# nihaomiao/CVPR23_LFDM

Measured on AMD Instinct MI355X. Metric: 40-frame 128x128 videos/sec (DDIM-100), higher is better.
Workload: dtype f32; 1 GPU; MUG 128x128, 40-frame DDIM-100 sample, batch=1 per GPU (BASELINE.json configs[1]); global_batch=1, frames=40, latent=32, image=128, sampler=DDIM-100 eta=1, cond_scale=1, parallelism=replicas x1 (videos sharded, no collective)

## Files before the change

cvpr23_lfdm_amd/_native.py:

```python
import ctypes as C
import os

_PKG_DIR = os.path.dirname(os.path.abspath(__file__))
HIP_LIB_PATH = os.environ.get("LFDM_HIP_LIB", os.path.join(_PKG_DIR, "liblfdm_hip.so"))

f32p = C.c_void_p
i32 = C.c_int
i64 = C.c_int64
f32 = C.c_float
sz = C.c_size_t
stream_t = C.c_void_p


class ConvParams(C.Structure):
    _fields_ = [
        ("src0", f32p), ("src1", f32p),
        ("c0", i32), ("c1", i32), ("ld0", i32), ("ld1", i32),
        ("n_img", i32), ("hi", i32), ("wi", i32),
        ("hq", i32), ("wq", i32),
        ("stride", i32), ("upsample", i32), ("pad_mode", i32),
        ("kh", i32), ("kw", i32), ("pad_y", i32), ("pad_x", i32),
        ("weight", f32p),
        ("cout", i32), ("coutp", i32),
        ("bias", f32p),
# ... 73 lines not shown
class WarpBwdParams(C.Structure):
    _fields_ = [
        ("src", f32p), ("dout", f32p), ("prev", f32p), ("dprev", f32p), ("dsrc_fix", C.c_void_p), ("amax_bits", C.c_void_p),
        ("dmaps", f32p), ("flow_x", f32p), ("flow_y", f32p), ("occ", f32p),
        ("n_img", i32), ("h", i32), ("w", i32), ("c", i32), ("fh", i32), ("fw", i32), ("n_div", i32), ("layout_cl", i32),
        ("fsn", i64),
        ("ld_src", i32), ("ld_dout", i32), ("ld_prev", i32), ("ld_dprev", i32),
        ("ss_n", i64), ("ss_c", i64), ("ss_h", i64), ("ss_w", i64), ("ds_n", i64), ("ds_c", i64), ("ds_h", i64), ("ds_w", i64),
        ("ps_n", i64), ("ps_c", i64), ("ps_h", i64), ("ps_w", i64), ("dps_n", i64), ("dps_c", i64), ("dps_h", i64), ("dps_w", i64),
    ]


class GridSampleParams(C.Structure):
    _fields_ = [
        ("x", f32p), ("grid", f32p), ("out", f32p), ("dout", f32p), ("dgrid", f32p),
        ("xs_n", i64), ("xs_c", i64), ("xs_h", i64), ("xs_w", i64), ("os_n", i64), ("os_c", i64), ("os_h", i64), ("os_w", i64),
        ("n_img", i32), ("channels", i32), ("h", i32), ("w", i32), ("ho", i32), ("wo", i32), ("n_div", i32), ("pad_mode", i32),
    ]


BN_TICKETS = 1024
OPTIM_PLAN_BYTES = 64

_SIGNATURES = {
    "lfdm_last_error": (C.c_char_p, []),
    "lfdm_abi_version": (i32, []),
    "lfdm_calib_mfma_f32": (i32, [f32p, i32, i32, stream_t]),
    "lfdm_conv2d_cl_f32": (i32, [C.POINTER(ConvParams), stream_t]),
    "lfdm_conv2d_cl_wino_bf16": (i32, [C.POINTER(ConvParams), C.c_void_p, stream_t]),
    "lfdm_conv2d_partial_bytes": (sz, [C.POINTER(ConvParams)]),
    "lfdm_conv2d_plan": (i32, [C.POINTER(ConvParams), C.POINTER(i32), C.POINTER(i32)]),
    "lfdm_conv2d_plan_slabs": (i32, [C.POINTER(ConvParams)]),
    "lfdm_conv2d_schedule": (i32, [C.POINTER(ConvParams)]),
    "lfdm_groupnorm_ws_bytes": (sz, [i32, i32, i32]),
    "lfdm_groupnorm_silu_cl_f32": (i32, [f32p, f32p, i32, i32, i32, i32, f32p, f32p, f32p, i32, f32p,
                                        f32, i32, C.c_void_p, sz, stream_t]),
    "lfdm_groupnorm_apply_cl_f32": (i32, [f32p, f32p, i32, i32, i32, i32, f32p, f32p, f32p, i32, f32p, f32, i32,
                                         f32p, i32, C.c_void_p, sz, stream_t]),
    "lfdm_layernorm_cl_f32": (i32, [f32p, f32p, i64, i32, f32p, f32, stream_t]),
    "lfdm_attention_cl_f32": (i32, [f32p, f32p, i32, i32, i32, i32, f32p, f32p, f32p, stream_t]),
    "lfdm_temporal_attention_fused_cl_f32": (i32, [f32p, i32, i32, f32p, f32p, i32, i32, i32, f32p, f32p, f32p, f32,
                                                  stream_t]),
    "lfdm_temporal_attention_fused_out_cl_f32": (i32, [f32p, i32, i32, f32p, f32p, f32p, i32, i32, i32, i32, f32p, f32p, f32p, f32,
                                                      stream_t]),
    "lfdm_linear_attention_lowres_cl_f32": (i32, [f32p, i32, i32, f32p, f32p, f32p, i32, i32, f32, stream_t]),
    "lfdm_attention_lowres_cl_f32": (i32, [f32p, i32, i32, f32p, f32p, f32p, i32, i32, i32, i32, f32p, f32p, f32p, f32, stream_t]),
    "lfdm_pack_wino_weight_f32": (i32, [f32p, i32, i32, i32, i32, i32, f32p, stream_t]),
    "lfdm_pack_wino4_weight_f32": (i32, [f32p, i32, i32, i32, i32, f32p, stream_t]),
    "lfdm_pack_wino_weight_bf16": (i32, [f32p, i32, i32, i32, i32, C.c_void_p, stream_t]),
    "lfdm_pack_conv_weight_f32": (i32, [f32p, i32, i32, i32, i64, i64, i32, f32p, stream_t]),
    "lfdm_lfae_motion_inputs_f32": (i32, [f32p, f32p, f32p, f32p, f32p, f32p, f32p, f32p, C.c_float, i32, i32, i32, i32, i32, i32,
                                          f32p, i32, f32p, stream_t]),
    "lfdm_lfae_region_stats_f32": (i32, [f32p, i32, i32, i32, i32, i32, C.c_float, f32p, f32p, f32p, f32p, f32p, f32p, stream_t]),
    "lfdm_svd2x2_sym_f32": (i32, [f32p, i64, f32p, f32p, stream_t]),
    "lfdm_lfae_motion_combine_f32": (i32, [f32p, i32, f32p, i32, i32, i32, f32p, f32p, stream_t]),
    "lfdm_conv2d_smalln_cl_f32": (i32, [f32p, i32, i32, i32, i32, i32, f32p, f32p, f32p, i32, i32, i32, i32, stream_t]),
    "lfdm_linear_attention_fused_ws_bytes": (sz, [i32, i32]),
    "lfdm_linear_attention_fused_cl_f32": (i32, [f32p, i32, i32, f32p, f32p, i32, i32, f32, C.c_void_p, sz, stream_t]),
    "lfdm_linear_attention_fused_out_cl_f32": (i32, [f32p, i32, i32, f32p, f32p, f32p, f32p, i32, i32, i32, f32, C.c_void_p, sz, stream_t]),
    "lfdm_linear_attention_ws_bytes": (sz, [i32]),
    "lfdm_linear_attention_cl_f32": (i32, [f32p, f32p, i32, i32, C.c_void_p, sz, stream_t]),
    "lfdm_linear_small_f32": (i32, [f32p, f32p, f32p, f32p, i32, i32, i32, i32, i32, i32, i32, i32, stream_t]),
    "lfdm_step_cond_f32": (i32, [f32p, f32p, C.c_void_p, f32p, i32, i32, stream_t]),
    "lfdm_sinusoidal_f32": (i32, [C.c_void_p, i32, f32p, f32p, i32, i32, i32, stream_t]),
    "lfdm_conv_planar_in_cl_f32": (i32, [f32p, i32, i32, i32, i32, i32, i32, f32p, i32, i32, i32,
                                        f32p, f32p, f32p, i32, i32, stream_t]),
# ... 121 lines not shown
```

cvpr23_lfdm_amd/csrc/conv_igemm.hip:

```cpp
#include <stdlib.h>

#include "lfdm_device.h"
#include "../../include/lfdm_hip.h"

namespace {

__device__ __forceinline__ bool src_pixel(const lfdm_conv_params& p, int img, int qy, int qx,
                                          int tap, int64_t& pix) {
  const int ky = tap / p.kw, kx = tap - ky * p.kw;
  int iy = qy * p.stride + ky - p.pad_y;
  int ix = qx * p.stride + kx - p.pad_x;
  const int H = p.upsample ? 2 * p.hi : p.hi;
  const int W = p.upsample ? 2 * p.wi : p.wi;
  if (p.pad_mode == 1) {
    if (iy < 0) iy = -iy;
    if (iy >= H) iy = 2 * (H - 1) - iy;
    if (ix < 0) ix = -ix;
    if (ix >= W) ix = 2 * (W - 1) - ix;
  } else if (iy < 0 || iy >= H || ix < 0 || ix >= W) {
    return false;
  }
  if (p.upsample) {
    iy >>= 1;
    ix >>= 1;
// ... 600 lines not shown
int splitk_col_chunks(const lfdm_conv_params& p, int64_t M) {
  const int c4n = p.coutp / 4;
  const int64_t rowblocks = (M + SPLITK_ROWS - 1) / SPLITK_ROWS;
  int gy = 1;
  while (rowblocks * gy < 256 && gy < 16) {
    const int cand = gy * 2;
    if (c4n % cand != 0) break;
    const int cw = c4n / cand;
    if (cw < 16) break;
    if (p.gn_partial) {
      const int cg4 = (p.cout / p.gn_groups) / 4;
      if (cw % cg4 != 0 || 256 % cw != 0) break;
    }
    gy = cand;
  }
  return gy;
}

template <int BM, int BN>
void launch_conv(const lfdm_conv_params& p, bool fast, bool simple, dim3 grid, hipStream_t stream) {
  dim3 block(256);
  if (fast && simple && p.ln_wsum) LFDM_LAUNCH((conv_igemm_kernel<BM, BN, true, true, true>), grid, block, 0, stream, p);
  else if (fast && simple) LFDM_LAUNCH((conv_igemm_kernel<BM, BN, true, true, false>), grid, block, 0, stream, p);
  else if (fast) LFDM_LAUNCH((conv_igemm_kernel<BM, BN, true, false, false>), grid, block, 0, stream, p);
  else LFDM_LAUNCH((conv_igemm_kernel<BM, BN, false, false, false>), grid, block, 0, stream, p);
}

}

int lfdm_conv_ksw_launch(const lfdm_conv_params& p, int bn, hipStream_t stream);
int lfdm_conv_wino_launch(const lfdm_conv_params& p, int bn, bool fuse_reduce, int bal_whole, hipStream_t stream);
int lfdm_conv_wino_bf16_launch(const lfdm_conv_params& p, const void* weight_bf16, int bn, bool fuse_reduce, int bal_whole, hipStream_t stream);
int lfdm_conv_pw_launch(const lfdm_conv_params& p, hipStream_t stream);
int lfdm_conv_wino4_launch(const lfdm_conv_params& p, hipStream_t stream);

namespace {

struct ConvPlan;
bool splitk_fused(const ConvPlan& pl, const lfdm_conv_params& p);
bool wino_fuse_geometry_ok(const lfdm_conv_params& p, int bn);
int wino_balance(const ConvPlan& pl, const lfdm_conv_params& p, int* extra_slabs);

struct ConvPlan {
  int kind;
  int bm, bn, ksplit;
  bool fast, simple;
};

int conv_force() {
  static int v = -2;
  if (v == -2) {
    const char* e = getenv("LFDM_CONV_FORCE");
    v = !e ? -1 : (e[0] == 'k' ? 1 : 0);
  }
  return v;
}

bool wino_enabled() {
  const char* e = getenv("LFDM_WINO");
  return !(e && e[0] == '0');
}

ConvPlan make_plan(const lfdm_conv_params& p) {
  ConvPlan pl;
  const int cin = p.c0 + p.c1;
  const int64_t M = (int64_t)p.n_img * p.hq * p.wq;
// ... 81 lines not shown
  if (ksw) {
    pl.kind = 1;
    pl.bm = 160;
    const int64_t mt = (M + 159) / 160 * (p.deconv4 ? 4 : 1);
    const int64_t t64 = mt * ((p.coutp + 63) / 64), t32 = mt * ((p.coutp + 31) / 32);
    pl.bn = (t64 >= 224 && p.coutp > 32) ? 64 : 32;
    int k = 1;
    if (t64 < 224 && t32 < 224) {
      k = (int)(256 / t32);
      if (k > nchunks / 4) k = nchunks / 4;
      if (k < 1) k = 1;
    }
    pl.ksplit = user_k >= 1 ? user_k : k;
  } else {
    pl.kind = 0;
    static const long wide_min = [] { const char* e = lfdm_knob("LFDM_IGEMM_WIDE_MIN"); return e ? atol(e) : 512l; }();
    const bool wide = p.coutp >= 128 && (M / 128) * (p.coutp / 128) >= wide_min;
    const bool small_m = M * (int64_t)((p.coutp + 63) / 64) < 128 * 512;
    pl.bm = wide ? 128 : (small_m ? 64 : 128);
    pl.bn = wide ? 128 : 64;
    int k = 1;
    const int64_t tiles = ((M + pl.bm - 1) / pl.bm) * ((p.coutp + pl.bn - 1) / pl.bn) * (p.deconv4 ? 4 : 1);
    if (tiles < 256 && nchunks >= 8) {
      k = (int)(512 / tiles);
      if (k > nchunks / 4) k = nchunks / 4;
      if (k > 16) k = 16;
      if (k < 1) k = 1;
    }
    pl.ksplit = user_k >= 1 ? user_k : k;
  }
  if (pl.ksplit > nchunks) pl.ksplit = nchunks;
  if (pl.ksplit < 1) pl.ksplit = 1;
  const int64_t pw_rows = (!p.ln_wsum && p.c0 + p.c1 <= 256 && p.coutp <= 128) ? 10240 : 1024;
  if (pwg_ok || (pw_ok && (pw_mode == 2 || M <= pw_rows || pl.ksplit > 1 || p.res_gn_partial))) {
    pl.kind = 3;
    pl.bm = 32;
    pl.bn = 32;
    pl.ksplit = 1;
  }
  return pl;
}

bool wino_fuse_geometry_ok(const lfdm_conv_params& p, int bn) {
  static const bool on = [] { const char* e = getenv("LFDM_WINO_FUSE_REDUCE"); return !(e && e[0] == '0'); }();
  if (!on || !p.tile_counters || p.deconv4 || bn != 32 || p.groups > 1 || p.pool2 || p.cout != p.coutp || p.ldo % 4 != 0 ||
      (((uintptr_t)p.out) & 15) != 0 ||
      (p.bias && (((uintptr_t)p.bias) & 15) != 0) ||
      (p.residual && (p.ldr % 4 != 0 || (((uintptr_t)p.residual) & 15) != 0)))
    return false;
  const int64_t ntiles = (int64_t)p.n_img * (p.hq / 2) * (p.wq / 2);
  return (int64_t)p.tile_counters_len >= ((ntiles + 31) / 32) * (p.coutp / 32);
}

bool splitk_fused(const ConvPlan& pl, const lfdm_conv_params& p) {
  if (pl.ksplit <= 1 || pl.kind != 2 || !wino_fuse_geometry_ok(p, pl.bn)) return false;
  const int64_t M = (int64_t)p.n_img * p.hq * p.wq;
  return (int64_t)pl.ksplit * M * p.coutp * 4 < (1ll << 32) - 64;
}

int wino_balance(const ConvPlan& pl, const lfdm_conv_params& p, int* extra_slabs) {
  if (extra_slabs) *extra_slabs = 0;
  static const bool on = [] { const char* e = getenv("LFDM_WINO_BALANCE"); return !(e && e[0] == '0'); }();
  static const bool fuse_on = [] { const char* e = getenv("LFDM_WINO_FUSE_REDUCE"); return !(e && e[0] == '0'); }();
  if (!on || !fuse_on || pl.kind != 2 || pl.bn != 32 || !p.tile_counters || p.deconv4 || p.groups > 1 || p.pool2 || p.cout != p.coutp || p.ldo % 4 != 0 ||
      (((uintptr_t)p.out) & 15) != 0 || (p.bias && (((uintptr_t)p.bias) & 15) != 0) ||
      (p.residual && (p.ldr % 4 != 0 || (((uintptr_t)p.residual) & 15) != 0)))
    return 0;
  if (pl.ksplit > 1 && !splitk_fused(pl, p)) return 0;
  const int64_t ntiles = (int64_t)p.n_img * (p.hq / 2) * (p.wq / 2);
  const int64_t T = ((ntiles + 31) / 32) * (p.coutp / 32);
  const int whole = 512, jobs = 640;
  if (T * pl.ksplit != jobs || (int64_t)p.tile_counters_len < T) return 0;
  const int nch = (p.c0 + p.c1) / 16;
  if (nch / pl.ksplit < 2) return 0;
  const int z_first = T - 1 >= whole ? 0 : (int)((whole - (T - 1) + T - 1) / T);
  const int extra = pl.ksplit - z_first;
  if (extra < 1) return 0;
  const int64_t M = (int64_t)p.n_img * p.hq * p.wq;
  if ((int64_t)(pl.ksplit + extra) * M * p.coutp * 4 >= (1ll << 32) - 64) return 0;
  if (extra_slabs) *extra_slabs = extra;
  return whole;
}

}

extern "C" int lfdm_conv2d_plan(const lfdm_conv_params* p, int* tile_rows, int* ksplit) {
  if (!p) return LFDM_EINVAL;
  const ConvPlan pl = make_plan(*p);
  if (tile_rows) *tile_rows = (pl.ksplit > 1 && !splitk_fused(pl, *p)) ? SPLITK_ROWS : pl.bm;
  if (ksplit) *ksplit = pl.ksplit;
  return LFDM_OK;
}

extern "C" int lfdm_conv2d_schedule(const lfdm_conv_params* p) {
  if (!p) return LFDM_EINVAL;
  return make_plan(*p).kind;
}

extern "C" size_t lfdm_conv2d_partial_bytes(const lfdm_conv_params* p) {
  if (!p) return 0;
  const ConvPlan pl = make_plan(*p);
  int extra = 0;
  wino_balance(pl, *p, &extra);
  if (pl.ksplit <= 1 && extra == 0) return 0;
  const size_t rows = (size_t)p->n_img * p->hq * p->wq;
  return ((size_t)(pl.ksplit + extra) * (p->deconv4 ? 4 : 1) * rows * p->coutp + (p->ln_wsum ? (size_t)pl.ksplit * rows * 2 : 0)) * sizeof(float) + 128;
}

extern "C" int lfdm_conv2d_plan_slabs(const lfdm_conv_params* p) {
  if (!p) return LFDM_EINVAL;
  const ConvPlan pl = make_plan(*p);
  int extra = 0;
  wino_balance(pl, *p, &extra);
  return pl.ksplit + extra;
}

namespace {

int conv2d_run(const lfdm_conv_params* pp, const void* wino_bf16, hipStream_t stream) {
  if (!pp) { lfdm_set_error("conv2d: null params"); return LFDM_EINVAL; }
  lfdm_conv_params p = *pp;
  if (!p.src0 || !p.weight || !p.out || p.c0 <= 0 || p.c1 < 0 || (p.c1 > 0 && !p.src1) ||
      p.n_img <= 0 || p.hq <= 0 || p.wq <= 0 || p.kh <= 0 || p.kw <= 0 || p.cout <= 0 ||
      (int64_t)p.n_img * p.hq * p.wq >= (1ll << 31) || p.coutp < p.cout || (p.coutp % 32) != 0 || p.stride <= 0 || p.out_scale <= 0 || p.ksplit < 0 ||
      p.ld0 < p.c0 || (p.c1 > 0 && p.ld1 < p.c1) || p.ldo < p.cout) {
    lfdm_set_error("conv2d: invalid geometry");
    return LFDM_EINVAL;
  }
  if (p.pad_mode == 1) {
    const int H = p.upsample ? 2 * p.hi : p.hi, W = p.upsample ? 2 * p.wi : p.wi;
    if (p.pad_y >= H || p.pad_x >= W || p.kh - 1 - p.pad_y >= H || p.kw - 1 - p.pad_x >= W) {
// ... 117 lines not shown
```

cvpr23_lfdm_amd/csrc/conv_pw.hip:

```cpp
#include <stdlib.h>

#include "lfdm_device.h"
#include "../../include/lfdm_hip.h"

namespace {

template <int TN, int KW, bool LN, bool GATHER = false>
__global__ __launch_bounds__(256) void conv_pw_kernel(lfdm_conv_params p, int gx, int ny) {
  constexpr int NW = 4 / KW;
  constexpr int LD = 36;
  __shared__ __attribute__((aligned(16))) float scratch[4 * 32 * LD];
  __shared__ float s_ln[2][4][32];
  constexpr int BN = (4 / KW) * TN * 32;
  __shared__ __attribute__((aligned(16))) float s_ga[BN], s_gb[BN];
  __shared__ float s_gstat[2][64];

  const int tid = threadIdx.x, lane = tid & 63;
  const int wave = lfdm_uniform(tid >> 6);
  const int wk = wave % KW, wn = wave / KW;
  const int id = blockIdx.x, slot = id >> 3;
  const int bx = (id & 7) + 8 * (slot / ny), by = slot % ny;
  if (bx >= gx) return;
  const int M = p.n_img * p.hq * p.wq;
  const int m0 = bx * 32;
// ... 199 lines not shown
    for (int g = 0; g < NW; ++g) {
      float4 v = *reinterpret_cast<const float4*>(scratch + (g * KW) * (32 * LD) + trow * LD + 4 * c4);
#pragma unroll
      for (int k = 1; k < KW; ++k) {
        const float4 u = *reinterpret_cast<const float4*>(scratch + (g * KW + k) * (32 * LD) + trow * LD + 4 * c4);
        v.x += u.x; v.y += u.y; v.z += u.z; v.w += u.w;
      }
      const int col = n0 + (g * TN + j) * 32 + 4 * c4;
      if (!vec_row || col >= p.cout) continue;
      if (LN) {
        const float4 ws = pre_w[g * TN + j];
        v.x = rstd * (v.x - mean * ws.x); v.y = rstd * (v.y - mean * ws.y);
        v.z = rstd * (v.z - mean * ws.z); v.w = rstd * (v.w - mean * ws.w);
      }
      {
        const float4 bb = pre_b[g * TN + j];
        float4 rr = pre_r[g * TN + j];
        if (p.res_gn_partial) {
          const float4 ga = *reinterpret_cast<const float4*>(s_ga + col - n0), gb = *reinterpret_cast<const float4*>(s_gb + col - n0);
          rr.x = silu_fast_(fmaf(rr.x, ga.x, gb.x)); rr.y = silu_fast_(fmaf(rr.y, ga.y, gb.y));
          rr.z = silu_fast_(fmaf(rr.z, ga.z, gb.z)); rr.w = silu_fast_(fmaf(rr.w, ga.w, gb.w));
        }
        v.x += bb.x + rr.x; v.y += bb.y + rr.y; v.z += bb.z + rr.z; v.w += bb.w + rr.w;
      }
      if (p.act) {
        v.x = apply_act(v.x, p.act); v.y = apply_act(v.y, p.act);
        v.z = apply_act(v.z, p.act); v.w = apply_act(v.w, p.act);
      }
      *reinterpret_cast<float4*>(p.out + (int64_t)orow * p.ldo + col) = v;
    }
  }
}

template <int TN, int KW>
void launch_pw(const lfdm_conv_params& p, int gx, int ny, hipStream_t stream) {
  const dim3 grid((unsigned)(((gx + 7) / 8) * 8 * ny)), block(256);
  if (p.kh * p.kw > 1) {
    if constexpr (TN <= 2 && KW == 4) LFDM_LAUNCH((conv_pw_kernel<TN, 4, false, true>), grid, block, 0, stream, p, gx, ny);
    return;
  }
  if (p.ln_wsum) LFDM_LAUNCH((conv_pw_kernel<TN, KW, true>), grid, block, 0, stream, p, gx, ny);
  else LFDM_LAUNCH((conv_pw_kernel<TN, KW, false>), grid, block, 0, stream, p, gx, ny);
}

int env_int(const char* name, int dflt) {
  const char* e = lfdm_knob(name);
  return e ? atoi(e) : dflt;
}

}

void lfdm_conv_pw_shape(const lfdm_conv_params& p, int* tn, int* kw) {
  const int K = p.kh * p.kw > 1 ? p.kh * p.kw * p.c0 : p.c0 + p.c1;
  const int64_t M = (int64_t)p.n_img * p.hq * p.wq;
  if (p.kh * p.kw > 1) {
    *tn = (p.coutp % 64 == 0 && ((M + 31) / 32) * (p.coutp / 64) >= 256) ? 2 : 1;
    *kw = 4;
    return;
  }
  int k = K % 128 == 0 ? 4 : K % 64 == 0 ? 2 : 1;
  const int fk = env_int("LFDM_PW_KW", 0);
  if ((fk == 1 || fk == 2 || fk == 4) && K % (32 * fk) == 0) k = fk;
  int t = (M <= 1024 && p.coutp >= 768 && p.coutp % ((4 / k) * 96) == 0) ? 3 : 1;
  const int ft = env_int("LFDM_PW_TN", 0);
  if (ft >= 1 && ft <= 3) t = ft;
  *tn = t;
  *kw = k;
}

int lfdm_conv_pw_launch(const lfdm_conv_params& p, hipStream_t stream) {
  int tn, kw;
  lfdm_conv_pw_shape(p, &tn, &kw);
  const int64_t M = (int64_t)p.n_img * p.hq * p.wq;
  const int gx = (int)((M + 31) / 32);
  const int bn = (4 / kw) * tn * 32;
  const int ny = (p.coutp + bn - 1) / bn;
#define LFDM_PW_CASE(T, W) if (tn == T && kw == W) launch_pw<T, W>(p, gx, ny, stream)
  LFDM_PW_CASE(1, 4); else LFDM_PW_CASE(2, 4); else LFDM_PW_CASE(3, 4);
  else LFDM_PW_CASE(1, 2); else LFDM_PW_CASE(2, 2); else LFDM_PW_CASE(3, 2);
  else LFDM_PW_CASE(1, 1); else LFDM_PW_CASE(2, 1); else LFDM_PW_CASE(3, 1);
#undef LFDM_PW_CASE
  return lfdm_check_launch("conv_pw");
}
```

cvpr23_lfdm_amd/csrc/lfdm_device.h:

```cpp
#pragma once
#include <stddef.h>
#include <stdint.h>
#include <type_traits>

#if defined(LFDM_EMU_BUILD)
#include "hip_emu.h"
typedef emu_f32x16 f32x16;
typedef emu_f32x4 f32x4;
#define LFDM_LAUNCH(kern, grid, block, smem, stream, ...) \
  emu::launch(grid, block, smem, [=]() { kern(__VA_ARGS__); })
static inline f32x16 mfma_32x32x2(float a, float b, f32x16 c) { return emu_mfma_32x32x2(a, b, c); }
static inline f32x4 mfma_16x16x4(float a, float b, f32x4 c) { return emu_mfma_16x16x4(a, b, c); }
static inline f32x4 mfma_4x4x1(float a, float b, f32x4 c) { return emu_mfma_4x4x1(a, b, c); }
struct lfdm_bf16x8 { uint16_t h[8]; };
static inline uint16_t lfdm_f32_to_bf16(float f) {
  uint32_t u;
  memcpy(&u, &f, 4);
  if ((u & 0x7fffffffu) > 0x7f800000u) return (uint16_t)((u >> 16) | 0x40u);
  u += 0x7fffu + ((u >> 16) & 1u);
  return (uint16_t)(u >> 16);
}
static inline float lfdm_bf16_to_f32(uint16_t h) {
  const uint32_t u = (uint32_t)h << 16;
  float f;
// ... 85 lines not shown
  float4 v = make_float4(0.f, 0.f, 0.f, 0.f);
  if ((uint64_t)off + 16u <= (uint64_t)b.bytes) memcpy(&v, b.base + off, 16);
  return v;
}
static inline float2 lfdm_buf_load_f2(lfdm_buf b, uint32_t off) {
  float2 v = make_float2(0.f, 0.f);
  if ((uint64_t)off + 8u <= (uint64_t)b.bytes) memcpy(&v, b.base + off, 8);
  return v;
}
#else
typedef __amdgpu_buffer_rsrc_t lfdm_buf;
typedef int lfdm_i32x4 __attribute__((ext_vector_type(4)));
__device__ __forceinline__ lfdm_buf lfdm_make_buf(const void* p, uint32_t bytes) {
  return __builtin_amdgcn_make_buffer_rsrc(const_cast<void*>(p), 0, (int)bytes, 0x00020000);
}
__device__ __forceinline__ float4 lfdm_buf_load_f4(lfdm_buf b, uint32_t off) {
  const lfdm_i32x4 v = __builtin_amdgcn_raw_buffer_load_b128(b, (int)off, 0, 0);
  float4 f;
  f.x = __int_as_float(v.x);
  f.y = __int_as_float(v.y);
  f.z = __int_as_float(v.z);
  f.w = __int_as_float(v.w);
  return f;
}
typedef int lfdm_i32x2 __attribute__((ext_vector_type(2)));
__device__ __forceinline__ float2 lfdm_buf_load_f2(lfdm_buf b, uint32_t off) {
  const lfdm_i32x2 v = __builtin_amdgcn_raw_buffer_load_b64(b, (int)off, 0, 0);
  return make_float2(__int_as_float(v.x), __int_as_float(v.y));
}
#endif
#define LFDM_BUF_OOB 0xFFFFFFF0u

#if defined(LFDM_EMU_BUILD)
static inline void lfdm_buf_store_f4_sc1(lfdm_buf b, uint32_t off, float4 v) {
  if ((uint64_t)off + 16u <= (uint64_t)b.bytes) memcpy(const_cast<char*>(b.base) + off, &v, 16);
}
static inline float4 lfdm_buf_load_f4_sc1(lfdm_buf b, uint32_t off) { return lfdm_buf_load_f4(b, off); }
#else
__device__ __forceinline__ void lfdm_buf_store_f4_sc1(lfdm_buf b, uint32_t off, float4 v) {
  lfdm_i32x4 d;
  d.x = __float_as_int(v.x); d.y = __float_as_int(v.y); d.z = __float_as_int(v.z); d.w = __float_as_int(v.w);
  __builtin_amdgcn_raw_buffer_store_b128(d, b, (int)off, 0, 16);
}
__device__ __forceinline__ float4 lfdm_buf_load_f4_sc1(lfdm_buf b, uint32_t off) {
  const lfdm_i32x4 v = __builtin_amdgcn_raw_buffer_load_b128(b, (int)off, 0, 16);
  float4 f;
  f.x = __int_as_float(v.x); f.y = __int_as_float(v.y); f.z = __int_as_float(v.z); f.w = __int_as_float(v.w);
  return f;
}
#endif

#if defined(LFDM_EMU_BUILD)
template <int OFF = 0> static inline void lfdm_gload_f4(f32x4& dst, const float* p) { memcpy(&dst, (const char*)p + OFF, 16); }
template <int N> static inline void lfdm_vmwait() {}
template <int N> static inline void lfdm_vmwait(f32x4&) {}
template <int N> static inline void lfdm_vmwait(f32x4&, f32x4&) {}
template <int N> static inline void lfdm_vmwait(f32x4&, f32x4&, f32x4&, f32x4&) {}
static inline void lfdm_tie(f32x4&) {}
static inline int lfdm_uniform(int v) { return v; }
#else
template <int OFF = 0>
__device__ __forceinline__ void lfdm_gload_f4(f32x4& dst, const float* p) {
  asm volatile("global_load_dwordx4 %0, %1, off offset:%2" : "=v"(dst) : "v"(p), "n"(OFF) : "memory");
}
template <int N> __device__ __forceinline__ void lfdm_vmwait() { asm volatile("s_waitcnt vmcnt(%0)" ::"n"(N) : "memory"); }
template <int N> __device__ __forceinline__ void lfdm_vmwait(f32x4& a) { asm volatile("s_waitcnt vmcnt(%1)" : "+v"(a) : "n"(N) : "memory"); }
// ... 99 lines not shown
```

cvpr23_lfdm_amd/ops.py:

```python
import ctypes as C

import torch

from . import _native
from ._native import ConvParams, WarpParams

ACT_NONE, ACT_RELU, ACT_SIGMOID, ACT_SILU, ACT_GELU = 0, 1, 2, 3, 4


def _lib():
    return _native.library()


def _stream(lib):
    if lib.kind == "hip":
        return C.c_void_p(torch.cuda.current_stream().cuda_stream)
    return None


def _p(t):
    return None if t is None else C.c_void_p(t.data_ptr())


def _chk(lib, *tensors):
# ... 306 lines not shown
        _chk(lib, gp, gg, gb)
        assert residual is not None and gg.numel() == cout == gb.numel() and gp.is_contiguous()
        p.res_gn_partial, p.res_gn_nchunk, p.res_gn_groups, p.res_gn_pixels = _p(gp), int(res_gn["nchunk"]), int(res_gn.get("groups", 8)), int(res_gn["pixels"])
        p.res_gn_gamma, p.res_gn_beta, p.res_gn_eps = _p(gg), _p(gb), float(res_gn.get("eps", 1e-5))
        keep_gn = keep_gn + (gp, gg, gb)
    p.pool2 = int(bool(pool2))
    p._keep = (src0, src1, weight, bias, residual, out, ln_wsum, tile_counters, weight_wino, deconv4, weight_wino4) + keep_gn
    return p, out


def conv_partial_floats(p):
    return _lib().lfdm_conv2d_partial_bytes(C.byref(p)) // 4


def conv_plan_slabs(p):
    return _lib().lfdm_conv2d_plan_slabs(C.byref(p))


class WinogradUnavailable(RuntimeError):
    pass


def conv_plan(p):
    lib = _lib()
    rows, ks = C.c_int(0), C.c_int(0)
    lib.check(lib.lfdm_conv2d_plan(C.byref(p), C.byref(rows), C.byref(ks)), "lfdm_conv2d_plan")
    return rows.value, ks.value


def conv_schedule(p):
    return _lib().lfdm_conv2d_schedule(C.byref(p))


def conv_launch(p):
    lib = _lib()
    lib.check(lib.lfdm_conv2d_cl_f32(C.byref(p), _stream(lib)), "lfdm_conv2d_cl_f32")


def _chk_wino_bf16(lib, p, wwb):
    if wwb.dtype != torch.bfloat16 or not wwb.is_contiguous():
        raise TypeError("weight_wino_bf16: a contiguous torch.bfloat16 pack (pack_wino_weight_bf16) expected, got %s" % wwb.dtype)
    if (lib.kind == "hip") != wwb.is_cuda:
        raise RuntimeError("weight_wino_bf16 must live where the library runs (GPU for hip, CPU for emu)")
    ww = p._keep[8]
    if ww is None or tuple(wwb.shape) != tuple(ww.shape):
        raise ValueError("weight_wino_bf16 needs weight_wino (the fp32 pack that decides the plan) of the same shape")


def conv_launch_wino_bf16(p, weight_wino_bf16):
    lib = _lib()
    _chk_wino_bf16(lib, p, weight_wino_bf16)
    lib.check(lib.lfdm_conv2d_cl_wino_bf16(C.byref(p), _p(weight_wino_bf16), _stream(lib)), "lfdm_conv2d_cl_wino_bf16")


def conv2d_cl(src0, weight, cout, kh, kw, n_img, hi, wi, *, partial=None, gn_partial=None, gn_groups=8,
              gn_pixels=0, weight_wino_bf16=None, **kw_):
    lib = _lib()
    _chk(lib, partial, gn_partial)
    p, out = conv_params(src0, weight, cout, kh, kw, n_img, hi, wi, **kw_)
    if weight_wino_bf16 is not None:
        _chk_wino_bf16(lib, p, weight_wino_bf16)
        if kw_.get("pool2") or lib.lfdm_conv2d_schedule(C.byref(p)) != 2:
            raise WinogradUnavailable("bf16 operands exist on the Winograd F(2x2,3x3) schedule only, without pool2: the library would not run it "
                                      "for this geometry")
    if (weight is None or kw_.get("pool2")) and lib.lfdm_conv2d_schedule(C.byref(p)) not in ((2,) if kw_.get("pool2") else (2, 4)):
        raise WinogradUnavailable("the library would not run the Winograd schedule for this geometry: pass the direct-form pack / "
# ... 837 lines not shown
```

cvpr23_lfdm_amd/unet.py:

```python
import os

import torch
from torch import nn

from . import ops
from .params import ParamTree, build_tree, unet_spec, weights_epoch

BERT_MODEL_DIM = 768
MAX_FRAMES = 64


def check_num_frames(num_frames):
    if not 1 <= int(num_frames) <= MAX_FRAMES:
        raise ValueError("num_frames = %d: the temporal-attention kernels are built for 1 ... %d frames" % (int(num_frames), MAX_FRAMES))


_LOWRES_ATTN = os.environ.get("LFDM_LOWRES_ATTN", "1") != "0"
_LOWRES_MAX_HW = 64
_WINO_FUSE_REDUCE = os.environ.get("LFDM_WINO_FUSE_REDUCE", "1") != "0"
_TATTN_OUT = os.environ.get("LFDM_TATTN_OUT", "1") != "0"
_LINATTN_OUT = os.environ.get("LFDM_LINATTN_OUT", "1") != "0"
_RES_GN_MAX_ROWS = 65536
_RES_GN = os.environ.get("LFDM_RES_GN", "1") != "0"
_HEADS_GN = os.environ.get("LFDM_HEADS_GN", "1") != "0"
# ... 244 lines not shown
            out[pk["heads.block2.ww"].data_ptr()] = ops.pack_wino_weight_grouped_bf16([g(h + "block2.proj.weight")[:, :, 0] for h in hp])
        return out

    def _tables(self, pk, frames):
        t = pk["tables"].get(frames)
        if t is None:
            bias = rel_pos_bias_table(pk["rel_emb"], frames)
            ang = torch.arange(frames, device=bias.device).float()[:, None] * pk["freqs"][None, :]
            t = (bias, ang.cos().contiguous(), ang.sin().contiguous())
            pk["tables"][frames] = t
        return t

    def time_embedding(self, pk, t_dev, batch, t_stride=1):
        e = ops.sinusoidal(t_dev, pk["time.freqs"], batch, self.dim, t_stride=t_stride)
        e = ops.linear_small(e, pk["time.w1"], pk["time.b1"], act_out=ops.ACT_GELU)
        return ops.linear_small(e, pk["time.w3"], pk["time.b3"])

    def merge_cond(self, cond, null_mask):
        null = self.null_cond_emb.to(cond.device, cond.dtype)
        return torch.where(null_mask.view(-1, 1), null, cond).contiguous()

    def cond_scale_shift(self, pk, temb, cond):
        tc = torch.cat((temb, cond), dim=-1).contiguous()
        return ops.linear_small(tc, pk["cond.w"], pk["cond.b"], act_in=ops.ACT_SILU)

    def cond_tables(self, pk, temb_steps, cond):
        td = temb_steps.shape[1]
        w = pk["cond.w"]
        step_part = ops.linear_small(temb_steps, w[:, :td], None, act_in=ops.ACT_SILU)
        sample_part = ops.linear_small(cond, w[:, td:], pk["cond.b"], act_in=ops.ACT_SILU)
        return step_part, sample_part

    def _conv(self, src0, w, cout, k, n_img, s, *, src1=None, bias=None, residual=None, out=None, gn=None,
              scratch="splitk", ww=None, **kw):
        if ((k == 1 or (k == 4 and kw.get("stride") == 2)) and self._pk is not None and w.dim() == 3 and w.shape[1] % 32 == 0 and
                not kw.get("deconv4")):
            cache = self._pk.setdefault("_pw", {})
            wpw = cache.get(w.data_ptr())
            if wpw is None:
                wpw = cache[w.data_ptr()] = ops.pack_pw_weight(w)
            kw["weight_pw"] = wpw
        p, y = ops.conv_params(src0, w, cout, k, k, n_img, s, s, src1=src1, bias=bias, residual=residual,
                               out=out, weight_wino=ww if (src1 is None or src0.shape[1] % 16 == 0) else None, **kw)
        coutp = p.coutp
        sched = ops.conv_schedule(p) if (_WINO_FUSE_REDUCE and kw.get("deconv4") is None) else -1
        if sched == 2:
            counters = self._tile_counters(src0.device)
            p.tile_counters, p.tile_counters_len = counters.data_ptr(), counters.numel()
        wwb = None
        if self._conv_precision == "bf16" and p.weight_wino is not None:
            wwb = self._pk["wino_bf16"][ww.data_ptr()]
        if gn is not None:
            p.gn_partial = 1
        tile_rows, ksplit = ops.conv_plan(p)
        partial_floats = ops.conv_partial_floats(p) if (ksplit > 1 or sched == 2) else 0
        p.gn_partial = None
        m = n_img * p.hq * p.wq
        if partial_floats > 0:
            part = self._buf(scratch, 1, partial_floats)
            p.partial = part.data_ptr()
        stats = None
        if gn is not None:
            batch, groups = gn[0], (gn[1] if len(gn) > 1 else 8)
            pixels = m // batch
            cg = cout // groups
            fused = ksplit > 1 and tile_rows != 16
            parts = cg // 32 if (fused and tile_rows == 128 and cg > 32 and cg % 32 == 0) else 1
            in_tile = (ksplit == 1 or fused) and (32 % cg == 0 or parts > 1)
            in_reduce = ksplit > 1 and not fused and 256 % (coutp // 4) == 0 and coutp == cout
            if pixels % tile_rows == 0 and cg % 4 == 0 and (in_tile or in_reduce):
                nchunk = pixels // tile_rows * (parts if in_tile else 1)
                stats = (self._buf("gn.partial", batch * nchunk, 2 * groups), nchunk)
                p.gn_partial, p.gn_groups, p.gn_pixels = stats[0].data_ptr(), groups, pixels
        if wwb is not None and ops.conv_schedule(p) == 2:
            ops.conv_launch_wino_bf16(p, wwb)
        else:
            ops.conv_launch(p)
        return (y, stats) if gn is not None else y

    def _tile_counters(self, dev):
        cur = getattr(self, "_tile_cnt", None)
        if cur is None or cur.device != torch.device(dev):
            cur = self._tile_cnt = torch.zeros(8192, dtype=torch.int32, device=dev)
            self._buf_gen += 1
        return cur

    def _gn(self, x, batch, gamma, beta, stats, groups=8, **kw):
        gws = self._buf("gn.ws", batch, 256 * 128 + 2 * 1024)
        if stats is not None:
            return ops.groupnorm_apply_cl(x, batch, gamma, beta, stats[0], stats[1], out=x, ws=gws, groups=groups, **kw)
        return ops.groupnorm_silu_cl(x, batch, gamma, beta, out=x, ws=gws, groups=groups, **kw)

    def _resblock(self, pk, prefix, x, skip, batch, frames, s, ss, cout, outname):
        n_img, rows = batch * frames, batch * frames * s * s
        h1 = self._buf("rb.h1", rows, cout)
        _, st = self._conv(x, pk[prefix + "block1.proj.w"], cout, 3, n_img, s, src1=skip,
                           bias=pk[prefix + "block1.proj.b"], out=h1, gn=(batch,), ww=pk[prefix + "block1.proj.ww"])
        sshift = None
        if ss is not None and (prefix + "ss_off") in pk:
            o = pk[prefix + "ss_off"]
            sshift = ss[:, o:o + 2 * cout]
        self._gn(h1, batch, pk[prefix + "block1.norm.w"], pk[prefix + "block1.norm.b"], st, scale_shift=sshift)
        out = self._buf(outname, rows, cout)
        _, st = self._conv(h1, pk[prefix + "block2.proj.w"], cout, 3, n_img, s, bias=pk[prefix + "block2.proj.b"],
                           out=out, gn=(batch,), ww=pk[prefix + "block2.proj.ww"])
        has_res = (prefix + "res.w") in pk
        if has_res and _RES_GN and st is not None and rows <= _RES_GN_MAX_ROWS and (rows // batch) % 32 == 0 and cout % 32 == 0:
            res_gn = dict(partial=st[0], nchunk=st[1], pixels=rows // batch, gamma=pk[prefix + "block2.norm.w"], beta=pk[prefix + "block2.norm.b"], groups=8)
            try:
                return self._conv(x, pk[prefix + "res.w"], cout, 1, n_img, s, src1=skip, bias=pk[prefix + "res.b"], residual=out, out=out,
                                  res_gn=res_gn)
            except RuntimeError:
                pass
        self._gn(out, batch, pk[prefix + "block2.norm.w"], pk[prefix + "block2.norm.b"], st,
                 residual=None if has_res else x)
        if has_res:
            self._conv(x, pk[prefix + "res.w"], cout, 1, n_img, s, src1=skip, bias=pk[prefix + "res.b"],
                       residual=out, out=out)
        return out

    def _attn_common(self, pk, prefix, x, n_img, s, c):
        rows = n_img * s * s
        qkv = self._buf("at.qkv", rows, 768)
        self._conv(x, pk[prefix + "qkv.w"], 768, 1, n_img, s, out=qkv, ln_wsum=pk[prefix + "qkv.wsum"])
        return qkv, self._buf("at.o", rows, 256)

    def _temporal_attn(self, pk, prefix, x, batch, frames, s, c, outname, tables, focus=None):
        bias, cos, sin = tables
        if focus is not None and any(focus):
            qkv, att = self._attn_common(pk, prefix, x, batch * frames, s, c)
            if not all(focus):
                ops.attention_cl(qkv, batch, frames, s * s, 0, bias=bias, rot_cos=cos, rot_sin=sin, out=att)
            out = self._buf(outname, x.shape[0], c)
            rows = frames * s * s
            for b in range(batch):
                sl = slice(b * rows, (b + 1) * rows)
                src = qkv[sl, 512:768] if focus[b] else att[sl]
                self._conv(src, pk[prefix + "out.w"], c, 1, frames, s, residual=x[sl], out=out[sl])
            return out
        if c == 64 and frames <= 64 and _TATTN_OUT:
            return ops.temporal_attention_fused_out_cl(x, pk[prefix + "qkv.wp"], pk[prefix + "out.wp"], batch, frames, s * s, bias=bias,
                                                       rot_cos=cos, rot_sin=sin, out=self._buf(outname, x.shape[0], c))
        if c == 64 and frames <= 64:
            att = self._buf("at.o", x.shape[0], 256)
            ops.temporal_attention_fused_cl(x, pk[prefix + "qkv.wf"], batch, frames, s * s, bias=bias, rot_cos=cos,
                                            rot_sin=sin, out=att)
# ... 178 lines not shown
```

include/lfdm_hip.h:

```cpp
#ifndef LFDM_HIP_H
#define LFDM_HIP_H

#include <stddef.h>
#include <stdint.h>

#ifdef __cplusplus
extern "C" {
#endif

typedef void* lfdm_stream_t;

#define LFDM_OK 0
#define LFDM_EINVAL (-1)
#define LFDM_ELAUNCH (-2)
#define LFDM_EWORKSPACE (-3)

#define LFDM_ACT_NONE 0
#define LFDM_ACT_RELU 1
#define LFDM_ACT_SIGMOID 2
#define LFDM_ACT_SILU 3
#define LFDM_ACT_GELU 4

const char* lfdm_last_error(void);
int lfdm_abi_version(void);
// ... 20 lines not shown
  int ksplit;
  float* partial;
  float* gn_partial;
  int gn_groups, gn_pixels;
  const float* ln_wsum;
  float ln_eps;
  unsigned int* tile_counters;
  int tile_counters_len;
  const float* weight_wino;
  int deconv4;
  int groups;
  int pool2;
  const float* weight_wino4;
  int defer_reduce;
  const float* weight_pw;
  const float* gn_in_partial;
  int gn_in_nchunk, gn_in_groups, gn_in_pixels;
  const float* gn_in_gamma;
  const float* gn_in_beta;
  const float* gn_in_ss;
  int gn_in_ss_ld;
  float gn_in_eps;
  const float* res_gn_partial;
  int res_gn_nchunk, res_gn_groups, res_gn_pixels;
  const float* res_gn_gamma;
  const float* res_gn_beta;
  float res_gn_eps;
} lfdm_conv_params;

int lfdm_conv2d_cl_f32(const lfdm_conv_params* p, lfdm_stream_t stream);
int lfdm_conv2d_cl_wino_bf16(const lfdm_conv_params* p, const void* weight_wino_bf16, lfdm_stream_t stream);
int lfdm_conv2d_plan(const lfdm_conv_params* p, int* tile_rows, int* ksplit);
int lfdm_conv2d_schedule(const lfdm_conv_params* p);
size_t lfdm_conv2d_partial_bytes(const lfdm_conv_params* p);
int lfdm_conv2d_plan_slabs(const lfdm_conv_params* p);

size_t lfdm_groupnorm_ws_bytes(int batch, int pixels, int channels);
int lfdm_groupnorm_silu_cl_f32(const float* x, float* out, int batch, int pixels, int channels,
                               int groups, const float* gamma, const float* beta,
                               const float* scale_shift, int ss_ld, const float* residual,
                               float eps, int apply_silu, void* ws, size_t ws_bytes,
                               lfdm_stream_t stream);

int lfdm_groupnorm_apply_cl_f32(const float* x, float* out, int batch, int pixels, int channels,
                                int groups, const float* gamma, const float* beta,
                                const float* scale_shift, int ss_ld, const float* residual,
                                float eps, int apply_silu, const float* partial, int nchunk,
                                void* ws, size_t ws_bytes, lfdm_stream_t stream);

int lfdm_layernorm_cl_f32(const float* x, float* out, int64_t rows, int channels,
                          const float* gamma, float eps, lfdm_stream_t stream);

int lfdm_attention_cl_f32(const float* qkv, float* out, int batch, int frames, int hw, int mode,
                          const float* bias, const float* rot_cos, const float* rot_sin,
                          lfdm_stream_t stream);

size_t lfdm_linear_attention_ws_bytes(int n_frames);
int lfdm_linear_attention_cl_f32(const float* qkv, float* out, int n_frames, int hw,
                                 void* ws, size_t ws_bytes, lfdm_stream_t stream);

int lfdm_linear_small_f32(const float* x, const float* w, const float* bias, float* y,
                          int batch, int k, int n, int ldx, int ldw, int ldy, int act_in,
                          int act_out, lfdm_stream_t stream);

int lfdm_step_cond_f32(const float* step_table, const float* batch_base, const int32_t* step_dev,
                       float* out, int batch, int n, lfdm_stream_t stream);
// ... 330 lines not shown
```

Baseline: 4.130 videos/s.

## Add persistent streaming pointwise conv kernel with register-resident weights

Adds a persistent 1x1-conv kernel for K in {64,96,128} and cout up to 128. Each block keeps its whole weight slice in registers, loops over row units with a capped grid, and prefetches the next unit's activations while MFMAs run. It can also fold the fused residual GroupNorm+SiLU path into the same kernel. The planner now routes large-M pointwise convs to this path, and the Python res-GN call checks the schedule instead of relying on a caught exception. The risks are lower occupancy from the large register footprint and per-block GN stat recomputation.

Result: no change. 4.137 videos/s, median of 5 (+0.2%).

```diff
diff --git a/cvpr23_lfdm_amd/_native.py b/cvpr23_lfdm_amd/_native.py
--- a/cvpr23_lfdm_amd/_native.py
+++ b/cvpr23_lfdm_amd/_native.py
@@ -129,6 +129,7 @@
     "lfdm_conv2d_plan": (i32, [C.POINTER(ConvParams), C.POINTER(i32), C.POINTER(i32)]),
     "lfdm_conv2d_plan_slabs": (i32, [C.POINTER(ConvParams)]),
     "lfdm_conv2d_schedule": (i32, [C.POINTER(ConvParams)]),
+    "lfdm_conv2d_pw_stream_rows": (i32, [C.POINTER(ConvParams)]),
     "lfdm_groupnorm_ws_bytes": (sz, [i32, i32, i32]),
     "lfdm_groupnorm_silu_cl_f32": (i32, [f32p, f32p, i32, i32, i32, i32, f32p, f32p, f32p, i32, f32p,
                                         f32, i32, C.c_void_p, sz, stream_t]),
diff --git a/cvpr23_lfdm_amd/csrc/conv_igemm.hip b/cvpr23_lfdm_amd/csrc/conv_igemm.hip
--- a/cvpr23_lfdm_amd/csrc/conv_igemm.hip
+++ b/cvpr23_lfdm_amd/csrc/conv_igemm.hip
@@ -656,6 +656,7 @@
 int lfdm_conv_wino_launch(const lfdm_conv_params& p, int bn, bool fuse_reduce, int bal_whole, hipStream_t stream);
 int lfdm_conv_wino_bf16_launch(const lfdm_conv_params& p, const void* weight_bf16, int bn, bool fuse_reduce, int bal_whole, hipStream_t stream);
 int lfdm_conv_pw_launch(const lfdm_conv_params& p, hipStream_t stream);
+int lfdm_conv_pw_stream_rows(const lfdm_conv_params& p);
 int lfdm_conv_wino4_launch(const lfdm_conv_params& p, hipStream_t stream);
 
 namespace {
@@ -803,7 +804,7 @@
   if (pl.ksplit > nchunks) pl.ksplit = nchunks;
   if (pl.ksplit < 1) pl.ksplit = 1;
   const int64_t pw_rows = (!p.ln_wsum && p.c0 + p.c1 <= 256 && p.coutp <= 128) ? 10240 : 1024;
-  if (pwg_ok || (pw_ok && (pw_mode == 2 || M <= pw_rows || pl.ksplit > 1 || p.res_gn_partial))) {
+  if (pwg_ok || (pw_ok && (pw_mode == 2 || M <= pw_rows || pl.ksplit > 1 || p.res_gn_partial || lfdm_conv_pw_stream_rows(p) > 0))) {
     pl.kind = 3;
     pl.bm = 32;
     pl.bn = 32;
@@ -868,6 +869,11 @@
   return make_plan(*p).kind;
 }
 
+extern "C" int lfdm_conv2d_pw_stream_rows(const lfdm_conv_params* p) {
+  if (!p) return LFDM_EINVAL;
+  return make_plan(*p).kind == 3 ? lfdm_conv_pw_stream_rows(*p) : 0;
+}
+
 extern "C" size_t lfdm_conv2d_partial_bytes(const lfdm_conv_params* p) {
   if (!p) return 0;
   const ConvPlan pl = make_plan(*p);
diff --git a/cvpr23_lfdm_amd/csrc/conv_pw.hip b/cvpr23_lfdm_amd/csrc/conv_pw.hip
--- a/cvpr23_lfdm_amd/csrc/conv_pw.hip
+++ b/cvpr23_lfdm_amd/csrc/conv_pw.hip
@@ -255,6 +255,159 @@
   }
 }
 
+constexpr int PWS_MAX_STATS = 256;
+
+template <int G>
+__global__ __launch_bounds__(256) void conv_pw_stream_kernel(lfdm_conv_params p, int nt, int units) {
+  __shared__ float s_gmean[PWS_MAX_STATS], s_grstd[PWS_MAX_STATS];
+  const int tid = threadIdx.x, lane = tid & 63;
+  const int wave = lfdm_uniform(tid >> 6);
+  const int ct = wave % nt, rsub = wave / nt, rw = 4 / nt;
+  int unit = blockIdx.x;
+  if (unit >= units) return;
+  const int M = p.n_img * p.hq * p.wq;
+  const int l31 = lane & 31, kh = lane >> 5;
+  const lfdm_buf buf0 = lfdm_make_buf(p.src0, (uint32_t)(((int64_t)(M - 1) * p.ld0 + p.c0) * 4));
+  const lfdm_buf buf1 = p.c1 > 0 ? lfdm_make_buf(p.src1, (uint32_t)(((int64_t)(M - 1) * p.ld1 + p.c1) * 4)) : buf0;
+  const lfdm_buf bufw = lfdm_make_buf(p.weight_pw, (uint32_t)((int64_t)G * p.coutp * 128));
+  const lfdm_buf bufo = lfdm_make_buf(p.out, (uint32_t)(((int64_t)(M - 1) * p.ldo + p.cout) * 4));
+  const lfdm_buf bufr = lfdm_make_buf(p.residual ? p.residual : p.out, p.residual ? (uint32_t)(((int64_t)(M - 1) * p.ldr + p.cout) * 4) : 0u);
+  const int col = ct * 32 + l31;
+  const bool col_ok = col < p.cout;
+
+  float4 rb[G][4];
+  {
+    const uint32_t wgroup_bytes = (uint32_t)p.coutp * 128u;
+    const bool tile_ok = ct * 32 < p.coutp;
+#pragma unroll
+    for (int g = 0; g < G; ++g)
+#pragma unroll
+      for (int u = 0; u < 4; ++u)
+        rb[g][u] = lfdm_buf_load_f4(bufw, tile_ok ? (uint32_t)g * wgroup_bytes + (uint32_t)ct * 4096u + 1024u * u + (uint32_t)lane * 16u : LFDM_BUF_OOB);
+  }
+
+  float4 ra[G][4];
+  auto fetch = [&](int s, int g, uint32_t off0, uint32_t off1, bool ok) {
+    const int kk = 32 * g;
+    const bool second = kk >= p.c0;
+    const lfdm_buf buf = second ? buf1 : buf0;
+    const uint32_t abase = second ? off1 + (uint32_t)(kk - p.c0) * 4u : off0 + (uint32_t)kk * 4u;
+#pragma unroll
+    for (int u = 0; u < 4; ++u) ra[s][u] = lfdm_buf_load_f4(buf, ok ? abase + 32u * u : LFDM_BUF_OOB);
+  };
+  int m0 = (unit * rw + rsub) * 32;
+  {
+    const int row = m0 + l31;
+    const uint32_t off0 = ((uint32_t)row * (uint32_t)p.ld0 + 4u * kh) * 4u, off1 = ((uint32_t)row * (uint32_t)p.ld1 + 4u * kh) * 4u;
+#pragma unroll
+    for (int g = 0; g < G; ++g) fetch(g, g, off0, off1, row < M);
+  }
+  const float bias_v = (p.bias && col_ok) ? p.bias[col] : 0.f;
+  float gn_gamma = 0.f, gn_beta = 0.f;
+  int gn_g = 0;
+  if (p.res_gn_partial) {
+    const int groups = p.res_gn_groups, nchunk = p.res_gn_nchunk, cg = p.cout / groups;
+    const int npairs = (M / p.res_gn_pixels) * groups;
+    const int sub = tid & 31;
+    gn_gamma = p.res_gn_gamma[col_ok ? col : 0];
+    gn_beta = p.res_gn_beta[col_ok ? col : 0];
+    gn_g = (col_ok ? col : 0) / cg;
+    for (int p0 = 0; p0 < npairs; p0 += 8) {
+      const int pr = p0 + (tid >> 5);
+      const bool pr_ok = pr < npairs;
+      double sm = 0.0, sq = 0.0;
+      if (pr_ok) {
+        const int b = pr / groups, g = pr - b * groups;
+        const float2* src = reinterpret_cast<const float2*>(p.res_gn_partial) + ((int64_t)b * nchunk) * groups + g;
+        int k = sub;
+        for (; k + 96 < nchunk; k += 128) {
+          const float2 v0 = src[(int64_t)k * groups], v1 = src[(int64_t)(k + 32) * groups];
+          const float2 v2 = src[(int64_t)(k + 64) * groups], v3 = src[(int64_t)(k + 96) * groups];
+          sm += (double)v0.x; sq += (double)v0.y;
+          sm += (double)v1.x; sq += (double)v1.y;
+          sm += (double)v2.x; sq += (double)v2.y;
+          sm += (double)v3.x; sq += (double)v3.y;
+        }
+        for (; k < nchunk; k += 32) {
+          const float2 v = src[(int64_t)k * groups];
+          sm += (double)v.x;
+          sq += (double)v.y;
+        }
+      }
+      for (int msk = 16; msk >= 1; msk >>= 1) {
+        sm += __shfl_xor(sm, msk);
+        sq += __shfl_xor(sq, msk);
+      }
+      if (pr_ok && sub == 0) {
+        const double n = (double)p.res_gn_pixels * (double)cg;
+        const double mean = sm / n;
+        double var = sq / n - mean * mean;
+        if (var < 0.0) var = 0.0;
+        s_gmean[pr] = (float)mean;
+        s_grstd[pr] = (float)(1.0 / sqrt(var + (double)p.res_gn_eps));
+      }
+    }
+    __syncthreads();
+  }
+
+  for (;;) {
+    const int next = unit + (int)gridDim.x;
+    const bool has_next = next < units;
+    const int m0n = ((has_next ? next : unit) * rw + rsub) * 32;
+    const int rown = m0n + l31;
+    const bool okn = rown < M;
+    const uint32_t off0n = ((uint32_t)rown * (uint32_t)p.ld0 + 4u * kh) * 4u, off1n = ((uint32_t)rown * (uint32_t)p.ld1 + 4u * kh) * 4u;
+    float rr[16];
+#pragma unroll
+    for (int r = 0; r < 16; ++r) {
+      const int orow = m0 + (r & 3) + 8 * (r >> 2) + 4 * kh;
+      rr[r] = lfdm_buf_load_f1(bufr, (col_ok && orow < M) ? ((uint32_t)orow * (uint32_t)p.ldr + (uint32_t)col) * 4u : LFDM_BUF_OOB);
+    }
+    f32x16 acc;
+#pragma unroll
+    for (int r = 0; r < 16; ++r) acc[r] = 0.f;
+#pragma unroll
+    for (int g = 0; g < G; ++g) {
+      float4 a[4];
+#pragma unroll
+      for (int u = 0; u < 4; ++u) a[u] = ra[g][u];
+      fetch(g, g, off0n, off1n, okn);
+#pragma unroll
+      for (int u = 0; u < 4; ++u) {
+        acc = mfma_32x32x2(a[u].x, rb[g][u].x, acc);
+        acc = mfma_32x32x2(a[u].y, rb[g][u].y, acc);
+        acc = mfma_32x32x2(a[u].z, rb[g][u].z, acc);
+        acc = mfma_32x32x2(a[u].w, rb[g][u].w, acc);
+      }
+    }
+    if (p.res_gn_partial) {
+      const int nb = M / p.res_gn_pixels;
+      int b = m0 / p.res_gn_pixels;
+      if (b >= nb) b = nb - 1;
+      const int pr = b * p.res_gn_groups + gn_g;
+      const float ga = s_grstd[pr] * gn_gamma;
+      const float gb = gn_beta - s_gmean[pr] * ga;
+#pragma unroll
+      for (int r = 0; r < 16; ++r) rr[r] = silu_fast_(fmaf(rr[r], ga, gb));
+    }
+    float v[16];
+#pragma unroll
+    for (int r = 0; r < 16; ++r) v[r] = acc[r] + (bias_v + rr[r]);
+    if (p.act) {
+#pragma unroll
+      for (int r = 0; r < 16; ++r) v[r] = apply_act(v[r], p.act);
+    }
+#pragma unroll
+    for (int r = 0; r < 16; ++r) {
+      const int orow = m0 + (r & 3) + 8 * (r >> 2) + 4 * kh;
+      lfdm_buf_store_f1(bufo, (col_ok && orow < M) ? ((uint32_t)orow * (uint32_t)p.ldo + (uint32_t)col) * 4u : LFDM_BUF_OOB, v[r]);
+    }
+    if (!has_next) break;
+    unit = next;
+    m0 = m0n;
+  }
+}
+
 template <int TN, int KW>
 void launch_pw(const lfdm_conv_params& p, int gx, int ny, hipStream_t stream) {
   const dim3 grid((unsigned)(((gx + 7) / 8) * 8 * ny)), block(256);
@@ -291,7 +444,33 @@
   *kw = k;
 }
 
+int lfdm_conv_pw_stream_rows(const lfdm_conv_params& p) {
+  if (p.kh * p.kw > 1 || !p.weight_pw || p.ln_wsum) return 0;
+  const int K = p.c0 + p.c1;
+  if ((K != 64 && K != 96 && K != 128) || p.coutp > 128 || K * p.coutp > 8192) return 0;
+  const int64_t M = (int64_t)p.n_img * p.hq * p.wq;
+  if (M * p.ldo * 4 >= (1ll << 32) - 64 || (p.residual && M * p.ldr * 4 >= (1ll << 32) - 64)) return 0;
+  if (p.res_gn_partial && (p.res_gn_pixels <= 0 || p.res_gn_groups <= 0 || (M / p.res_gn_pixels) * p.res_gn_groups > PWS_MAX_STATS)) return 0;
+  const int mode = env_int("LFDM_PW_STREAM", -1);
+  if (mode == 0 || (mode != 1 && M < 10240)) return 0;
+  return p.coutp <= 32 ? 128 : p.coutp <= 64 ? 64 : 32;
+}
+
 int lfdm_conv_pw_launch(const lfdm_conv_params& p, hipStream_t stream) {
+  if (const int span = lfdm_conv_pw_stream_rows(p)) {
+    const int64_t M = (int64_t)p.n_img * p.hq * p.wq;
+    const int K = p.c0 + p.c1, nt = 128 / span;
+    const int units = (int)((M + span - 1) / span);
+    int cap = 256;
+    const int fc = env_int("LFDM_PW_STREAM_GRID", 0);
+    if (fc > 0) cap = fc;
+    const int trips = (units + cap - 1) / cap;
+    const dim3 grid((unsigned)((units + trips - 1) / trips)), block(256);
+    if (K == 64) LFDM_LAUNCH((conv_pw_stream_kernel<2>), grid, block, 0, stream, p, nt, units);
+    else if (K == 96) LFDM_LAUNCH((conv_pw_stream_kernel<3>), grid, block, 0, stream, p, nt, units);
+    else LFDM_LAUNCH((conv_pw_stream_kernel<4>), grid, block, 0, stream, p, nt, units);
+    return lfdm_check_launch("conv_pw_stream");
+  }
   int tn, kw;
   lfdm_conv_pw_shape(p, &tn, &kw);
   const int64_t M = (int64_t)p.n_img * p.hq * p.wq;
diff --git a/cvpr23_lfdm_amd/csrc/lfdm_device.h b/cvpr23_lfdm_amd/csrc/lfdm_device.h
--- a/cvpr23_lfdm_amd/csrc/lfdm_device.h
+++ b/cvpr23_lfdm_amd/csrc/lfdm_device.h
@@ -141,6 +141,24 @@
 #define LFDM_BUF_OOB 0xFFFFFFF0u
 
 #if defined(LFDM_EMU_BUILD)
+static inline float lfdm_buf_load_f1(lfdm_buf b, uint32_t off) {
+  float v = 0.f;
+  if ((uint64_t)off + 4u <= (uint64_t)b.bytes) memcpy(&v, b.base + off, 4);
+  return v;
+}
+static inline void lfdm_buf_store_f1(lfdm_buf b, uint32_t off, float v) {
+  if ((uint64_t)off + 4u <= (uint64_t)b.bytes) memcpy(const_cast<char*>(b.base) + off, &v, 4);
+}
+#else
+__device__ __forceinline__ float lfdm_buf_load_f1(lfdm_buf b, uint32_t off) {
+  return __int_as_float(__builtin_amdgcn_raw_buffer_load_b32(b, (int)off, 0, 0));
+}
+__device__ __forceinline__ void lfdm_buf_store_f1(lfdm_buf b, uint32_t off, float v) {
+  __builtin_amdgcn_raw_buffer_store_b32(__float_as_int(v), b, (int)off, 0, 0);
+}
+#endif
+
+#if defined(LFDM_EMU_BUILD)
 static inline void lfdm_buf_store_f4_sc1(lfdm_buf b, uint32_t off, float4 v) {
   if ((uint64_t)off + 16u <= (uint64_t)b.bytes) memcpy(const_cast<char*>(b.base) + off, &v, 16);
 }
diff --git a/cvpr23_lfdm_amd/ops.py b/cvpr23_lfdm_amd/ops.py
--- a/cvpr23_lfdm_amd/ops.py
+++ b/cvpr23_lfdm_amd/ops.py
@@ -362,6 +362,10 @@
     return _lib().lfdm_conv2d_schedule(C.byref(p))
 
 
+def conv_pw_stream_rows(p):
+    return _lib().lfdm_conv2d_pw_stream_rows(C.byref(p))
+
+
 def conv_launch(p):
     lib = _lib()
     lib.check(lib.lfdm_conv2d_cl_f32(C.byref(p), _stream(lib)), "lfdm_conv2d_cl_f32")
diff --git a/cvpr23_lfdm_amd/unet.py b/cvpr23_lfdm_amd/unet.py
--- a/cvpr23_lfdm_amd/unet.py
+++ b/cvpr23_lfdm_amd/unet.py
@@ -300,7 +300,7 @@
         return step_part, sample_part
 
     def _conv(self, src0, w, cout, k, n_img, s, *, src1=None, bias=None, residual=None, out=None, gn=None,
-              scratch="splitk", ww=None, **kw):
+              scratch="splitk", ww=None, require_schedule=None, **kw):
         if ((k == 1 or (k == 4 and kw.get("stride") == 2)) and self._pk is not None and w.dim() == 3 and w.shape[1] % 32 == 0 and
                 not kw.get("deconv4")):
             cache = self._pk.setdefault("_pw", {})
@@ -310,6 +310,8 @@
             kw["weight_pw"] = wpw
         p, y = ops.conv_params(src0, w, cout, k, k, n_img, s, s, src1=src1, bias=bias, residual=residual,
                                out=out, weight_wino=ww if (src1 is None or src0.shape[1] % 16 == 0) else None, **kw)
+        if require_schedule is not None and ops.conv_schedule(p) != require_schedule:
+            return None
         coutp = p.coutp
         sched = ops.conv_schedule(p) if (_WINO_FUSE_REDUCE and kw.get("deconv4") is None) else -1
         if sched == 2:
@@ -375,11 +377,10 @@
         has_res = (prefix + "res.w") in pk
         if has_res and _RES_GN and st is not None and rows <= _RES_GN_MAX_ROWS and (rows // batch) % 32 == 0 and cout % 32 == 0:
             res_gn = dict(partial=st[0], nchunk=st[1], pixels=rows // batch, gamma=pk[prefix + "block2.norm.w"], beta=pk[prefix + "block2.norm.b"], groups=8)
-            try:
-                return self._conv(x, pk[prefix + "res.w"], cout, 1, n_img, s, src1=skip, bias=pk[prefix + "res.b"], residual=out, out=out,
-                                  res_gn=res_gn)
-            except RuntimeError:
-                pass
+            y = self._conv(x, pk[prefix + "res.w"], cout, 1, n_img, s, src1=skip, bias=pk[prefix + "res.b"], residual=out, out=out,
+                           res_gn=res_gn, require_schedule=3)
+            if y is not None:
+                return y
         self._gn(out, batch, pk[prefix + "block2.norm.w"], pk[prefix + "block2.norm.b"], st,
                  residual=None if has_res else x)
         if has_res:
diff --git a/include/lfdm_hip.h b/include/lfdm_hip.h
--- a/include/lfdm_hip.h
+++ b/include/lfdm_hip.h
@@ -76,6 +76,7 @@
 int lfdm_conv2d_cl_wino_bf16(const lfdm_conv_params* p, const void* weight_wino_bf16, lfdm_stream_t stream);
 int lfdm_conv2d_plan(const lfdm_conv_params* p, int* tile_rows, int* ksplit);
 int lfdm_conv2d_schedule(const lfdm_conv_params* p);
+int lfdm_conv2d_pw_stream_rows(const lfdm_conv_params* p);
 size_t lfdm_conv2d_partial_bytes(const lfdm_conv_params* p);
 int lfdm_conv2d_plan_slabs(const lfdm_conv_params* p);
 
```
